# TUMFTM/CamRaDepth

Measured on AMD Instinct MI355X. Metric: training images/sec at 256x416 bf16, higher is better.
Workload: dtype bf16; 1 GPU; CamRaDepth base (image+radar) train step, 8x7x256x416 per GPU, bf16 MFMA / fp32 accumulate, diffGradNorm + OneCycleLR, Dropout2d/DropPath on; global_batch=8, parallelism=dp1, hip_graph=True

## Files before the change

camradepth_amd/csrc/encoder_ops.hip:

```cpp
#include <stdlib.h>
#include "common.h"

namespace {

constexpr int TPB = 256;

constexpr int DTH = 8;
constexpr int DCW = 64;

struct InNorm {
  const crd_sum_t* stats;
  const float* gamma; const float* beta; int gmul;
};
__device__ __forceinline__ void innorm_coeffs(const InNorm& n, int b, int C, long long P, int c0, bool ok, float (&a)[8], float (&s)[8]) {
#pragma unroll
  for (int j = 0; j < 8; ++j) { a[j] = 1.f; s[j] = 0.f; }
  if (n.stats == nullptr || !ok) return;
  float mean, rstd;
  const int grp = (c0 >> 4) / n.gmul;
  gn_mean_rstd(n.stats + (long long)b * (C >> 4) * 2, grp * n.gmul, n.gmul, (float)P * 16.f * n.gmul, mean, rstd);
#pragma unroll
  for (int j = 0; j < 8; ++j) {
    a[j] = n.gamma[c0 + j] * rstd;
    s[j] = n.beta[c0 + j] - mean * a[j];
// ... 32 lines not shown
  bf16_t* yb = y + (long long)b * H * W * C;
  const int t = threadIdx.x;
  const int nG = (C - c_win) >= DCW ? 8 : (C - c_win) >> 3;
  const int g = t & 7, xc = (t >> 3) % TW, rg = (t >> 3) / TW;
  const int c0 = c_win + g * 8;
  const bool gok = g < nG;
  typedef __attribute__((ext_vector_type(2))) float f32x2;
  f32x2 wv[9][4], bv[4];
  {
    uint4 r[(HPX * 8 + TPB - 1) / TPB];
    bool inimg[(HPX * 8 + TPB - 1) / TPB];
#pragma unroll
    for (int k = 0; k < (HPX * 8 + TPB - 1) / TPB; ++k) {
      const int i = t + k * TPB;
      const int hp = i >> 3, g = i & 7;
      const int hy = hp / HWD, hx = hp - hy * HWD;
      const int iy = ty0 - 1 + hy, ix = tx0 - 1 + hx;
      inimg[k] = i < HPX * 8 && g < nG && (unsigned)iy < (unsigned)H && (unsigned)ix < (unsigned)W;
      const int cy = iy < 0 ? 0 : (iy < H ? iy : H - 1), cx = ix < 0 ? 0 : (ix < W ? ix : W - 1), cgr = g < nG ? g : 0;
      const uint4 u = *reinterpret_cast<const uint4*>(xb + ((long long)cy * W + cx) * C + c_win + cgr * 8);
      r[k] = inimg[k] ? u : make_uint4(0, 0, 0, 0);
    }
#pragma unroll
    for (int tp = 0; tp < 9; ++tp) {
      float w8[8];
      if (gok) load8t<1>(w9, (long long)(FLIP ? 8 - tp : tp) * C + c0, w8);
      else {
#pragma unroll
        for (int j = 0; j < 8; ++j) w8[j] = 0.f;
      }
#pragma unroll
      for (int q = 0; q < 4; ++q) wv[tp][q] = f32x2{w8[2 * q], w8[2 * q + 1]};
    }
#pragma unroll
    for (int q = 0; q < 4; ++q) bv[q] = f32x2{(bias && gok) ? bias[c0 + 2 * q] : 0.f, (bias && gok) ? bias[c0 + 2 * q + 1] : 0.f};
    float na[8], ns[8];
    innorm_coeffs(inn, b, C, (long long)H * W, c_win + (t & 7) * 8, (t & 7) < nG, na, ns);
#pragma unroll
    for (int k = 0; k < (HPX * 8 + TPB - 1) / TPB; ++k) {
      const int i = t + k * TPB;
      if (i < HPX * 8) sh[i] = (inn.stats && inimg[k]) ? innorm_apply(r[k], na, ns) : r[k];
    }
  }
  uint4 xrv[ROWS];
  if (red.xr) {
    const int cgr = gok ? c0 : c_win;
#pragma unroll
    for (int i = 0; i < ROWS; ++i) {
      const int oy = ty0 + rg * ROWS + i, ox = tx0 + xc;
      const int cy = oy < H ? oy : H - 1, cx = ox < W ? ox : W - 1;
      xrv[i] = *reinterpret_cast<const uint4*>(red.xr + (((long long)b * H + cy) * W + cx) * C + cgr);
    }
  }
  __syncthreads();
  auto lds8 = [&](int hy, int hx, f32x2 (&v)[4]) {
    const uint4 u = sh[(hy * HWD + hx) * 8 + g];
    v[0] = f32x2{bf_lo(u.x), bf_hi(u.x)}; v[1] = f32x2{bf_lo(u.y), bf_hi(u.y)};
    v[2] = f32x2{bf_lo(u.z), bf_hi(u.z)}; v[3] = f32x2{bf_lo(u.w), bf_hi(u.w)};
  };
  f32x2 win[3][3][4];
  const int r0 = rg * ROWS;
#pragma unroll
  for (int ky = 0; ky < 2; ++ky)
#pragma unroll
    for (int kx = 0; kx < 3; ++kx) lds8(r0 + ky, xc + kx, win[ky][kx]);
  float s = 0.f, ss = 0.f;
  float rs0[8], rs1[8], rmean = 0.f, rrstd = 0.f;
#pragma unroll
  for (int j = 0; j < 8; ++j) rs0[j] = rs1[j] = 0.f;
  if (red.xr && gok) gn_mean_rstd(red.stats + (long long)b * (C >> 4) * 2, c0 >> 4, 1, (float)H * W * 16.f, rmean, rrstd);
#pragma unroll
  for (int i = 0; i < ROWS; ++i) {
#pragma unroll
    for (int kx = 0; kx < 3; ++kx) lds8(r0 + i + 2, xc + kx, win[(i + 2) % 3][kx]);
    const int oy = ty0 + r0 + i, ox = tx0 + xc;
    f32x2 acc[4];
#pragma unroll
    for (int q = 0; q < 4; ++q) acc[q] = bv[q];
#pragma unroll
    for (int ky = 0; ky < 3; ++ky)
#pragma unroll
      for (int kx = 0; kx < 3; ++kx) {
#pragma unroll
        for (int q = 0; q < 4; ++q) acc[q] = __builtin_elementwise_fma(win[(i + ky) % 3][kx][q], wv[ky * 3 + kx][q], acc[q]);
      }
    if (gok && oy < H && ox < W) {
      uint4 u;
      u.x = pack_bf2(acc[0][0], acc[0][1]); u.y = pack_bf2(acc[1][0], acc[1][1]); u.z = pack_bf2(acc[2][0], acc[2][1]); u.w = pack_bf2(acc[3][0], acc[3][1]);
      *reinterpret_cast<uint4*>(yb + ((long long)oy * W + ox) * C + c0) = u;
      if (red.xr) {
        const uint4 xv = xrv[i];
        const float gq[8] = {bf_lo(u.x), bf_hi(u.x), bf_lo(u.y), bf_hi(u.y), bf_lo(u.z), bf_hi(u.z), bf_lo(u.w), bf_hi(u.w)};
        const float xq[8] = {bf_lo(xv.x), bf_hi(xv.x), bf_lo(xv.y), bf_hi(xv.y), bf_lo(xv.z), bf_hi(xv.z), bf_lo(xv.w), bf_hi(xv.w)};
#pragma unroll
        for (int j = 0; j < 8; ++j) { rs0[j] += gq[j]; rs1[j] += gq[j] * ((xq[j] - rmean) * rrstd); }
      }
      if (STATS) {
        s += bf_lo(u.x) + bf_hi(u.x) + bf_lo(u.y) + bf_hi(u.y) + bf_lo(u.z) + bf_hi(u.z) + bf_lo(u.w) + bf_hi(u.w);
        ss += bf_lo(u.x) * bf_lo(u.x) + bf_hi(u.x) * bf_hi(u.x) + bf_lo(u.y) * bf_lo(u.y) + bf_hi(u.y) * bf_hi(u.y) +
              bf_lo(u.z) * bf_lo(u.z) + bf_hi(u.z) * bf_hi(u.z) + bf_lo(u.w) * bf_lo(u.w) + bf_hi(u.w) * bf_hi(u.w);
      }
    }
  }
  if (STATS) {
    s += __shfl_xor(s, 1); ss += __shfl_xor(ss, 1);
#pragma unroll
    for (int o = 8; o < 64; o <<= 1) { s += __shfl_xor(s, o); ss += __shfl_xor(ss, o); }
    const int wave = t >> 6, l = t & 63;
    if (l < 8 && (l & 1) == 0) { sred[wave][(l >> 1) * 2] = s; sred[wave][(l >> 1) * 2 + 1] = ss; }
    __syncthreads();
    if (t < 8) {
      const float v = sred[0][t] + sred[1][t] + sred[2][t] + sred[3][t];
      const int slab = (c_win >> 4) + (t >> 1);
      if (slab < (C >> 4)) stat_add(&stats[((long long)b * (C >> 4) + slab) * 2 + (t & 1)], v);
    }
  }
  if (red.xr) {
#pragma unroll
    for (int o = 8; o < 64; o <<= 1) {
#pragma unroll
      for (int j = 0; j < 8; ++j) { rs0[j] += __shfl_xor(rs0[j], o); rs1[j] += __shfl_xor(rs1[j], o); }
    }
    __syncthreads();
    float* fr = reinterpret_cast<float*>(sh);
    const int wave = t >> 6, l = t & 63;
    if (l < 8) {
#pragma unroll
      for (int j = 0; j < 8; ++j) { fr[wave * 128 + (l * 8 + j) * 2] = rs0[j]; fr[wave * 128 + (l * 8 + j) * 2 + 1] = rs1[j]; }
    }
    __syncthreads();
    const int nch = nG * 8;
    if (t < 2 * nch) {
      const float v = fr[t] + fr[128 + t] + fr[256 + t] + fr[384 + t];
      const int c = c_win + (t >> 1);
      grad_add(&red.r[((long long)b * C + c) * 2 + (t & 1)], v);
      fr[512 + t] = v * red.gamma[c];
    }
    __syncthreads();
    if (t < 2 * (nch >> 4)) {
      const int grp = t >> 1, which = t & 1;
      float a = 0.f;
#pragma unroll
      for (int j = 0; j < 16; ++j) a += fr[512 + (grp * 16 + j) * 2 + which];
      grad_add(&red.r[(long long)gridDim.z * C * 2 + ((long long)b * (C >> 4) + (c_win >> 4) + grp) * 2 + which], a);
    }
  }
}

#ifndef CRD_DWW_WGS
#define CRD_DWW_WGS 2
#endif
template <int TW>
__global__ __launch_bounds__(TPB, CRD_DWW_WGS) void k_dwconv_wgrad(const bf16_t* x, const bf16_t* dy, int H, int W, int C, crd_sum_t* dw10,
                                                      int replicas, int tiles_x, int tiles_y, int tiles_per_wg, InNorm inn) {
  constexpr int HWD = TW + 2;
  constexpr int HPX = (DTH + 2) * HWD;
  constexpr int RSPLIT = 32 / TW;
  constexpr int ROWS = DTH / RSPLIT;
  extern __shared__ __attribute__((aligned(16))) uint4 dsm[];
  uint4* sx = dsm;
  uint4* sdy = dsm + HPX * 8;
  const int b = blockIdx.z;
  const int c_win = blockIdx.y * DCW;
  const int txi = blockIdx.x % tiles_x, ygrp = blockIdx.x / tiles_x;
  const int tx0 = txi * TW;
  const bf16_t* xb = x + (long long)b * H * W * C;
  const bf16_t* db = dy + (long long)b * H * W * C;
  const int t = threadIdx.x;
  const int nG = (C - c_win) >= DCW ? 8 : (C - c_win) >> 3;
  const int g = t & 7, xc = (t >> 3) % TW, rg = (t >> 3) / TW;
  float acc[10][8];
#pragma unroll
  for (int tp = 0; tp < 10; ++tp)
#pragma unroll
    for (int j = 0; j < 8; ++j) acc[tp][j] = 0.f;
  auto unpack8 = [&](const uint4& u, float (&v)[8]) {
    v[0] = bf_lo(u.x); v[1] = bf_hi(u.x); v[2] = bf_lo(u.y); v[3] = bf_hi(u.y);
    v[4] = bf_lo(u.z); v[5] = bf_hi(u.z); v[6] = bf_lo(u.w); v[7] = bf_hi(u.w);
  };
  float na[8], ns[8];
  for (int it = 0; it < tiles_per_wg; ++it) {
    const int tyi = ygrp * tiles_per_wg + it;
    if (tyi >= tiles_y) break;
    const int ty0 = tyi * DTH;
    {
      constexpr int NX = (HPX * 8 + TPB - 1) / TPB, ND = (DTH * TW * 8) / TPB;
      uint4 rx[NX], rd[ND];
      bool inimg[NX];
#pragma unroll
      for (int k = 0; k < NX; ++k) {
        const int i = t + k * TPB;
        const int hp = i >> 3, gg = i & 7;
        const int hy = hp / HWD, hx = hp - hy * HWD;
        const int iy = ty0 - 1 + hy, ix = tx0 - 1 + hx;
        inimg[k] = i < HPX * 8 && gg < nG && (unsigned)iy < (unsigned)H && (unsigned)ix < (unsigned)W;
        const int cy = iy < 0 ? 0 : (iy < H ? iy : H - 1), cx = ix < 0 ? 0 : (ix < W ? ix : W - 1), cgr = gg < nG ? gg : 0;
        const uint4 u = *reinterpret_cast<const uint4*>(xb + ((long long)cy * W + cx) * C + c_win + cgr * 8);
        rx[k] = inimg[k] ? u : make_uint4(0, 0, 0, 0);
      }
#pragma unroll
      for (int k = 0; k < ND; ++k) {
        const int i = t + k * TPB;
        const int pp = i >> 3, gg = i & 7;
        const int py = pp / TW, px = pp - py * TW;
        const int iy = ty0 + py, ix = tx0 + px;
        const int cy = iy < H ? iy : H - 1, cx = ix < W ? ix : W - 1, cgr = gg < nG ? gg : 0;
        const uint4 u = *reinterpret_cast<const uint4*>(db + ((long long)cy * W + cx) * C + c_win + cgr * 8);
        rd[k] = (gg < nG && iy < H && ix < W) ? u : make_uint4(0, 0, 0, 0);
      }
      if (it == 0) innorm_coeffs(inn, b, C, (long long)H * W, c_win + (t & 7) * 8, (t & 7) < nG, na, ns);
      if (it > 0) __syncthreads();
#pragma unroll
      for (int k = 0; k < NX; ++k) {
        const int i = t + k * TPB;
        if (i < HPX * 8) sx[i] = (inn.stats && inimg[k]) ? innorm_apply(rx[k], na, ns) : rx[k];
      }
#pragma unroll
      for (int k = 0; k < ND; ++k) sdy[t + k * TPB] = rd[k];
    }
    __syncthreads();
    float win[3][3][8];
    const int r0 = rg * ROWS;
#pragma unroll
    for (int ky = 0; ky < 2; ++ky)
#pragma unroll
      for (int kx = 0; kx < 3; ++kx) unpack8(sx[((r0 + ky) * HWD + xc + kx) * 8 + g], win[ky][kx]);
#pragma unroll
    for (int i = 0; i < ROWS; ++i) {
#pragma unroll
      for (int kx = 0; kx < 3; ++kx) unpack8(sx[((r0 + i + 2) * HWD + xc + kx) * 8 + g], win[(i + 2) % 3][kx]);
      float d[8];
      unpack8(sdy[((r0 + i) * TW + xc) * 8 + g], d);
#pragma unroll
      for (int j = 0; j < 8; ++j) acc[9][j] += d[j];
#pragma unroll
      for (int ky = 0; ky < 3; ++ky)
#pragma unroll
        for (int kx = 0; kx < 3; ++kx) {
#pragma unroll
          for (int j = 0; j < 8; ++j) acc[ky * 3 + kx][j] += d[j] * win[(i + ky) % 3][kx][j];
        }
    }
  }
#pragma unroll
  for (int o = 8; o < 64; o <<= 1) {
#pragma unroll
    for (int tp = 0; tp < 10; ++tp)
#pragma unroll
      for (int j = 0; j < 8; ++j) acc[tp][j] += __shfl_xor(acc[tp][j], o);
  }
  __syncthreads();
  float* sm = reinterpret_cast<float*>(dsm);
  const int wave = t >> 6, l = t & 63;
  for (int w = 0; w < 4; ++w) {
    if (wave == w && l < 8) {
#pragma unroll
      for (int tp = 0; tp < 10; ++tp)
#pragma unroll
        for (int j = 0; j < 8; ++j) {
          float* p = &sm[tp * 64 + l * 8 + j];
          *p = w == 0 ? acc[tp][j] : *p + acc[tp][j];
        }
    }
    __syncthreads();
  }
  crd_sum_t* dst = dw10 + (long long)((blockIdx.z * gridDim.x + blockIdx.x) % replicas) * 10 * C;
  const int nch = nG * 8;
  for (int i = t; i < 10 * nch; i += TPB) {
    const int tp = i / nch, cl = i - tp * nch;
    const float v = sm[tp * 64 + cl];
    if (v != 0.f) grad_add(&dst[(long long)tp * C + c_win + cl], v);
  }
}

template <class PRE, class F>
__device__ __forceinline__ void matvec_rows(const bf16_t* w, int ld, int r_lo, int r_hi, int ncols, const float* sx, PRE&& pre, F&& out) {
  const int l = threadIdx.x & 63, wave = threadIdx.x >> 6, nw = blockDim.x >> 6;
  auto load_rows = [&](int r0, int c0, float (&wv)[4][8]) {
#pragma unroll
    for (int k = 0; k < 4; ++k) {
      const int r = r0 + k < r_hi ? r0 + k : r_hi - 1;
      load8(w + (long long)r * ld, c0 < ncols ? c0 : 0, 0, wv[k]);
    }
  };
  float w0[4][8];
  const int r_first = r_lo + wave * 4;
  load_rows(r_first < r_hi ? r_first : r_lo, l * 8, w0);
  pre();
  for (int r0 = r_first; r0 < r_hi; r0 += nw * 4) {
    double acc[4] = {0.0, 0.0, 0.0, 0.0};
    for (int c0 = l * 8; c0 < ncols; c0 += 512) {
      float wv[4][8];
      if (r0 == r_first && c0 == l * 8) {
#pragma unroll
        for (int k = 0; k < 4; ++k)
#pragma unroll
          for (int j = 0; j < 8; ++j) wv[k][j] = w0[k][j];
      } else {
        load_rows(r0, c0, wv);
      }
#pragma unroll
      for (int k = 0; k < 4; ++k)
#pragma unroll
        for (int j = 0; j < 8; ++j) acc[k] += (double)wv[k][j] * (double)sx[c0 + j];
    }
#pragma unroll
    for (int k = 0; k < 4; ++k)
#pragma unroll
      for (int o = 32; o > 0; o >>= 1) acc[k] += __shfl_xor(acc[k], o);
    if (l == 0) {
#pragma unroll
      for (int k = 0; k < 4; ++k)
        if (r0 + k < r_hi) out(r0 + k, (float)acc[k]);
    }
  }
}
constexpr int VEC_ROWS = 64;

struct XbarProj { const crd_sum_t* chan; const crd_sum_t* stats; const float* gamma; const float* beta; const bf16_t* w; int N, C; bf16_t* xbar; float* u; };
__device__ __forceinline__ void attn_xbar_proj_body(const XbarProj& x, int b, int e) {
  __shared__ float sx[1024];
  const int C = x.C, N = x.N, nt = blockDim.x;
  const int r_lo = e * VEC_ROWS, r_hi = r_lo + VEC_ROWS < C ? r_lo + VEC_ROWS : C;
  float* ub = x.u + (long long)b * C;
  matvec_rows(x.w, C, r_lo, r_hi, C, sx,
              [&]() {
                for (int c = threadIdx.x; c < C; c += nt) {
                  float mean, rstd;
                  gn_mean_rstd(x.stats + (long long)b * (C >> 4) * 2, c >> 4, 1, (float)N * 16.f, mean, rstd);
                  const float mc = stat_get(&x.chan[((long long)b * C + c) * 2]) / (float)N;
                  const bf16_t q = f2bf(x.gamma[c] * (mc - mean) * rstd + x.beta[c]);
                  if (e == 0) x.xbar[(long long)b * C + c] = q;
                  sx[c] = bf2f(q);
                }
                __syncthreads();
              },
              [&](int r, float v) { ub[r] = v; });
}

__global__ __launch_bounds__(1024) void k_attn_scores(const bf16_t* q, const bf16_t* k, int N, int M, int heads, int d,
                                                      float scale, float* S, short* idx, int qg, XbarProj xp) {
  __shared__ float smax[16][32];
  const int b = blockIdx.y;
  const int nvec = xp.chan ? (xp.C + VEC_ROWS - 1) / VEC_ROWS : 0;
  if ((int)blockIdx.x < nvec) { attn_xbar_proj_body(xp, b, blockIdx.x); return; }
  const int tile_x = blockIdx.x - nvec;
  const int l = threadIdx.x & 63, wave = threadIdx.x >> 6;
  const int h = wave % heads, g = wave / heads;
  const int n0 = (tile_x * qg + g) * 32;
  const int C = heads * d;
  const int n = n0 + (l & 31);
  const bool nok = n < N;
  const bf16_t* qb = q + ((long long)b * N + (nok ? n : 0)) * C;
  const bf16_t* kb = k + (long long)b * M * C;
  const int half = l >> 5;
  bf16x8 qf[4];
#pragma unroll
  for (int ks = 0; ks < 4; ++ks) {
    const int kk = ks * 16 + half * 8;
    uint4 u = *reinterpret_cast<const uint4*>(qb + h * d + (kk < d ? kk : 0));
    if (kk >= d) u = make_uint4(0, 0, 0, 0);
    qf[ks] = *reinterpret_cast<bf16x8*>(&u);
  }
  float best = -INFINITY;
  int besti = 0;
  const bool kcol_ok[4] = {half * 8 < d, 16 + half * 8 < d, 32 + half * 8 < d, 48 + half * 8 < d};
  auto load_keys = [&](int m0, uint4 (&dst)[4]) {
    int mrow = m0 + (l & 31);
    mrow = mrow < M ? mrow : M - 1;
    const bf16_t* rowp = kb + (long long)mrow * C + h * d;
#pragma unroll
    for (int ks = 0; ks < 4; ++ks) dst[ks] = *reinterpret_cast<const uint4*>(rowp + (kcol_ok[ks] ? ks * 16 + half * 8 : 0));
  };
  auto score_tile = [&](int m0, const uint4 (&kt)[4]) {
    f32x16 acc;
#pragma unroll
    for (int r = 0; r < 16; ++r) acc[r] = 0.f;
#pragma unroll
    for (int ks = 0; ks < 4; ++ks) {
      uint4 kf = kt[ks];
      if (!kcol_ok[ks]) kf = make_uint4(0, 0, 0, 0);
      acc = __builtin_amdgcn_mfma_f32_32x32x16_bf16(*reinterpret_cast<const bf16x8*>(&kf), qf[ks], acc, 0, 0, 0);
    }
    const bool edge = m0 + 32 > M;
#pragma unroll
    for (int r = 0; r < 16; r += 2) {
      const int ma = m0 + (r & 3) + 8 * (r >> 2) + 4 * half;
      const uint32_t p1 = pack_bf2(acc[r], acc[r + 1]);
      const uint32_t p2 = pack_bf2(bf_lo(p1) * scale, bf_hi(p1) * scale);
      float va = bf_lo(p2), vb = bf_hi(p2);
      if (edge) { va = ma < M ? va : -INFINITY; vb = ma + 1 < M ? vb : -INFINITY; }
      const bool ta = va > best;
      best = ta ? va : best;
      besti = ta ? ma : besti;
      const bool tb = vb > best;
      best = tb ? vb : best;
      besti = tb ? ma + 1 : besti;
    }
  };
  uint4 ring[4][4];
#pragma unroll
  for (int j = 0; j < 4; ++j) load_keys(j * 32, ring[j]);
  for (int m0 = 0; m0 < M; m0 += 128) {
#pragma unroll
    for (int j = 0; j < 4; ++j) {
      score_tile(m0 + j * 32, ring[j]);
      __builtin_amdgcn_sched_barrier(0);
      load_keys(m0 + j * 32 + 128, ring[j]);
      __builtin_amdgcn_sched_barrier(0);
    }
  }
  float ob = __shfl_xor(best, 32);
  int oi = __shfl_xor(besti, 32);
  if (ob > best || (ob == best && oi < besti)) { best = ob; besti = oi; }
  if (nok && half == 0) idx[((long long)b * N + n) * heads + h] = (short)besti;
  if (half == 0) smax[wave][l] = best;
  __syncthreads();
  if (h == 0 && half == 0 && nok) {
    float Ssum = 0.f;
    for (int hh = 0; hh < heads; ++hh) Ssum += smax[g * heads + hh][l];
    S[(long long)b * N + n] = Ssum;
  }
}

// ... 251 lines not shown
  for (long long i0 = threadIdx.x; i0 < total; i0 += (long long)UB * TPB) {
    int cgv[UB], mv[UB];
    long long nv[UB];
    float gv[UB];
#pragma unroll
    for (int u = 0; u < UB; ++u) {
      const long long i = i0 + (long long)u * TPB;
      const bool ok = i < total;
      cgv[u] = ok ? (int)(i % CG) : 0;
      nv[u] = ok ? p0 + i / CG : p0;
      const int h = (cgv[u] * 8) / d;
      mv[u] = idx[((long long)b * N + nv[u]) * heads + h];
      gv[u] = ok ? scale * dS[(long long)b * N + nv[u]] : 0.f;
    }
    uint4 kraw[UB], qraw[UB];
#pragma unroll
    for (int u = 0; u < UB; ++u) {
      kraw[u] = *reinterpret_cast<const uint4*>(k + ((long long)b * M + mv[u]) * C + cgv[u] * 8);
      qraw[u] = *reinterpret_cast<const uint4*>(q + ((long long)b * N + nv[u]) * C + cgv[u] * 8);
    }
#pragma unroll
    for (int u = 0; u < UB; ++u) {
      if (i0 + (long long)u * TPB >= total) continue;
      float kv[8];
      kv[0] = bf_lo(kraw[u].x); kv[1] = bf_hi(kraw[u].x); kv[2] = bf_lo(kraw[u].y); kv[3] = bf_hi(kraw[u].y);
      kv[4] = bf_lo(kraw[u].z); kv[5] = bf_hi(kraw[u].z); kv[6] = bf_lo(kraw[u].w); kv[7] = bf_hi(kraw[u].w);
#pragma unroll
      for (int j = 0; j < 8; ++j) kv[j] *= gv[u];
      store8_bf16(dq, ((long long)b * N + nv[u]) * C + cgv[u] * 8, kv);
      if (use_lds) {
        const int nl = (int)(nv[u] - p0);
        sq[nl * CG + cgv[u]] = qraw[u];
        const int h = (cgv[u] * 8) / d;
        if (cgv[u] * 8 == h * d) atomicOr(&mask[(h * M + mv[u]) * WPC + (nl >> 5)], 1u << (nl & 31));
        if (cgv[u] == 0) sg[nl] = gv[u];
      } else {
        float qv[8];
        qv[0] = bf_lo(qraw[u].x); qv[1] = bf_hi(qraw[u].x); qv[2] = bf_lo(qraw[u].y); qv[3] = bf_hi(qraw[u].y);
        qv[4] = bf_lo(qraw[u].z); qv[5] = bf_hi(qraw[u].z); qv[6] = bf_lo(qraw[u].w); qv[7] = bf_hi(qraw[u].w);
        crd_sum_t* dst = &dk[((long long)b * M + mv[u]) * C + cgv[u] * 8];
#pragma unroll
        for (int j = 0; j < 8; ++j) grad_add(dst + j, gv[u] * qv[j]);
      }
    }
  }
  if (!use_lds) return;
  __syncthreads();
  float* outp = dk_part ? dk_part + ((long long)chunk_x * gridDim.y + b) * M * C : nullptr;
  for (int pr = threadIdx.x; pr < M * CG; pr += TPB) {
    const int m = pr / CG, cg = pr - m * CG;
    const int h = (cg * 8) / d;
    const unsigned* mk = mask + (h * M + m) * WPC;
    float acc[8];
#pragma unroll
    for (int j = 0; j < 8; ++j) acc[j] = 0.f;
    for (int w = 0; w < WPC; ++w) {
      unsigned bits = mk[w];
      while (bits) {
        const int n = (w << 5) + __builtin_ctz(bits);
        bits &= bits - 1;
        const uint4 u = sq[n * CG + cg];
        const float g = sg[n];
        acc[0] += g * bf_lo(u.x); acc[1] += g * bf_hi(u.x); acc[2] += g * bf_lo(u.y); acc[3] += g * bf_hi(u.y);
        acc[4] += g * bf_lo(u.z); acc[5] += g * bf_hi(u.z); acc[6] += g * bf_lo(u.w); acc[7] += g * bf_hi(u.w);
      }
    }
    if (outp) {
      store8_f32(outp, (long long)m * C + cg * 8, acc);
    } else {
      crd_sum_t* dst = &dk[((long long)b * M + m) * C + cg * 8];
#pragma unroll
      for (int j = 0; j < 8; ++j)
        if (acc[j] != 0.f) grad_add(dst + j, acc[j]);
    }
  }
}

__global__ __launch_bounds__(TPB) void k_sum_partials_bf16(const float* part, int replicas, long long stride, bf16_t* dst, long long n8) {
  for (long long i = (long long)blockIdx.x * TPB + threadIdx.x; i < n8; i += (long long)gridDim.x * TPB) {
    float v[8];
#pragma unroll
    for (int j = 0; j < 8; ++j) v[j] = 0.f;
    for (int r0 = 0; r0 < replicas; r0 += 4) {
      float w[4][8];
#pragma unroll
      for (int k = 0; k < 4; ++k) load8(part, (long long)(r0 + k < replicas ? r0 + k : replicas - 1) * stride + i * 8, 1, w[k]);
#pragma unroll
      for (int k = 0; k < 4; ++k) {
        const bool ok = r0 + k < replicas;
#pragma unroll
        for (int j = 0; j < 8; ++j) v[j] += ok ? w[k][j] : 0.f;
      }
    }
    store8_bf16(dst, i * 8, v);
  }
}

__global__ __launch_bounds__(TPB) void k_gsum_to_bf16(const crd_sum_t* src, bf16_t* dst, long long n8) {
  for (long long i = (long long)blockIdx.x * TPB + threadIdx.x; i < n8; i += (long long)gridDim.x * TPB) {
    float v[8];
#pragma unroll
    for (int j = 0; j < 8; ++j) v[j] = grad_get(src + i * 8 + j);
    store8_bf16(dst, i * 8, v);
  }
}

}

static int dw_tile_width(int W) {
  static int forced = -1;
  if (forced < 0) forced = crd_dev_int("CRD_DW_TW", 0);
  if (forced == 16 || forced == 32) return forced;
  return W <= 16 ? 16 : 32;
}

extern "C" int crd_dwconv3x3(const void* x, int32_t B, int32_t H, int32_t W, int32_t C, const float* w9, const float* bias,
                             int32_t flip, void* y, crd_sum_t* stats, const crd_sum_t* in_stats, int32_t in_gmul,
                             const float* in_gamma, const float* in_beta, const void* red_x, const crd_sum_t* red_stats,
                             const float* red_gamma, crd_sum_t* red_r, crd_stream_t stream) {
  CRD_CHECK_ARG(x && w9 && y, "crd_dwconv3x3: null pointer");
  CRD_CHECK_ARG(!red_x || (red_stats && red_gamma && red_r), "crd_dwconv3x3: incomplete fused-reduce arguments");
  const RedOut red{reinterpret_cast<const bf16_t*>(red_x), red_stats, red_gamma, red_r};
  CRD_CHECK_ARG(!in_stats || (in_gamma && in_beta && in_gmul >= 1 && (C / 16) % in_gmul == 0), "crd_dwconv3x3: bad input-norm arguments");
  const InNorm inn{in_stats, in_gamma, in_beta, in_gmul};
  CRD_CHECK_ARG(C % 16 == 0, "crd_dwconv3x3: C must be a multiple of 16");
  const bf16_t* xp = reinterpret_cast<const bf16_t*>(x);
  bf16_t* yp = reinterpret_cast<bf16_t*>(y);
  hipStream_t st = as_stream(stream);
  const int tw = dw_tile_width(W);
  const int tiles_x = cdiv(W, tw), tiles_y = cdiv(H, DTH);
  dim3 grid(tiles_x * tiles_y, cdiv(C, DCW), B);
#define CRD_DW(FL, STT, TWV) hipLaunchKernelGGL((k_dwconv<FL, STT, TWV>), grid, dim3(TPB), 0, st, xp, H, W, C, w9, bias, yp, stats, tiles_x, inn, red)
  if (tw == 32) {
    if (flip) { if (stats) CRD_DW(true, true, 32); else CRD_DW(true, false, 32); }
    else { if (stats) CRD_DW(false, true, 32); else CRD_DW(false, false, 32); }
  } else {
    if (flip) { if (stats) CRD_DW(true, true, 16); else CRD_DW(true, false, 16); }
    else { if (stats) CRD_DW(false, true, 16); else CRD_DW(false, false, 16); }
  }
#undef CRD_DW
  CRD_LAUNCH_CHECK("crd_dwconv3x3");
  return CRD_OK;
}

extern "C" int crd_dwconv3x3_wgrad(const void* x, const void* dy, int32_t B, int32_t H, int32_t W, int32_t C, crd_sum_t* dw10,
                                   int32_t replicas, const crd_sum_t* in_stats, int32_t in_gmul, const float* in_gamma,
                                   const float* in_beta, crd_stream_t stream) {
  CRD_CHECK_ARG(x && dy && dw10 && replicas >= 1, "crd_dwconv3x3_wgrad: null pointer / replicas < 1");
  CRD_CHECK_ARG(!in_stats || (in_gamma && in_beta && in_gmul >= 1 && (C / 16) % in_gmul == 0), "crd_dwconv3x3_wgrad: bad input-norm arguments");
  const InNorm inn{in_stats, in_gamma, in_beta, in_gmul};
  CRD_CHECK_ARG(C % 16 == 0 && C <= 4096, "crd_dwconv3x3_wgrad: C must be a multiple of 16, <= 4096");
  const int tw = dw_tile_width(W);
  const int tiles_x = cdiv(W, tw), tiles_y = cdiv(H, DTH), wins = cdiv(C, DCW);
  int ysplit = cdiv(512, (long long)tiles_x * wins * B);
  if (ysplit > tiles_y) ysplit = tiles_y;
  if (ysplit < 1) ysplit = 1;
  const int per = cdiv(tiles_y, ysplit);
  ysplit = cdiv(tiles_y, per);
  dim3 grid(tiles_x * ysplit, wins, B);
  const bf16_t* xp = reinterpret_cast<const bf16_t*>(x);
  const bf16_t* dp = reinterpret_cast<const bf16_t*>(dy);
  hipStream_t st = as_stream(stream);
  static bool attr_done[2] = {false, false};
  if (tw == 32) {
    const size_t lds = (size_t)((DTH + 2) * 34 * 8 + DTH * 32 * 8) * sizeof(uint4);
    if (!attr_done[0]) { crd_reserve_lds(reinterpret_cast<const void*>(&k_dwconv_wgrad<32>), (int)lds, "k_dwconv_wgrad"); attr_done[0] = true; }
    hipLaunchKernelGGL(k_dwconv_wgrad<32>, grid, dim3(TPB), lds, st, xp, dp, H, W, C, dw10, replicas, tiles_x, tiles_y, per, inn);
  } else {
    const size_t lds = (size_t)((DTH + 2) * 18 * 8 + DTH * 16 * 8) * sizeof(uint4);
    if (!attr_done[1]) { crd_reserve_lds(reinterpret_cast<const void*>(&k_dwconv_wgrad<16>), (int)lds, "k_dwconv_wgrad"); attr_done[1] = true; }
    hipLaunchKernelGGL(k_dwconv_wgrad<16>, grid, dim3(TPB), lds, st, xp, dp, H, W, C, dw10, replicas, tiles_x, tiles_y, per, inn);
  }
  CRD_LAUNCH_CHECK("crd_dwconv3x3_wgrad");
  return CRD_OK;
}

static int attn_scores_launch(const void* q, const void* k, int32_t B, int32_t N, int32_t M, int32_t heads, int32_t d, float scale,
                              float* S, int16_t* idx, const XbarProj& xp, const char* who, crd_stream_t stream) {
  CRD_CHECK_ARG(q && k && S && idx, "%s: null pointer", who);
  CRD_UNSUPPORTED(d % 8 == 0 && d <= 64 && M < 32768, "%s: head dim must be a multiple of 8, <= 64 (got %d)", who, d);
  CRD_UNSUPPORTED(heads >= 1 && heads <= 16, "%s: at most 16 heads (got %d)", who, heads);
  int qg = 8 / heads;
  if (qg < 1) qg = 1;
  if (qg > 4) qg = 4;
  dim3 grid(cdiv(N, 32 * qg) + (xp.chan ? cdiv(xp.C, VEC_ROWS) : 0), B);
  hipLaunchKernelGGL(k_attn_scores, grid, dim3(64 * heads * qg), 0, as_stream(stream), reinterpret_cast<const bf16_t*>(q),
                     reinterpret_cast<const bf16_t*>(k), N, M, heads, d, scale, S, idx, qg, xp);
  CRD_LAUNCH_CHECK(who);
  return CRD_OK;
}

extern "C" int crd_attn_scores(const void* q, const void* k, int32_t B, int32_t N, int32_t M, int32_t heads, int32_t d,
                               float scale, float* S, int16_t* idx, crd_stream_t stream) {
  return attn_scores_launch(q, k, B, N, M, heads, d, scale, S, idx, XbarProj{}, "crd_attn_scores", stream);
}

extern "C" int crd_attn_scores_fp8(const void* q8, const void* k8, int32_t B, int32_t N, int32_t M, int32_t heads, float qk_scale,
                                   float scale, float* ssum, int16_t* idx, crd_stream_t stream) {
  CRD_CHECK_ARG(q8 && k8 && ssum && idx && B > 0 && N > 0 && M > 0 && qk_scale > 0.f, "crd_attn_scores_fp8: bad argument");
  CRD_UNSUPPORTED(heads >= 1 && heads <= 16, "crd_attn_scores_fp8: at most 16 heads");
  CRD_CHECK_ARG((reinterpret_cast<uintptr_t>(q8) & 15) == 0 && (reinterpret_cast<uintptr_t>(k8) & 15) == 0, "crd_attn_scores_fp8: 16-byte aligned operands");
  int qg = 8 / heads;
  if (qg < 1) qg = 1;
  if (qg > 4) qg = 4;
  hipLaunchKernelGGL(k_attn_scores_fp8, dim3(cdiv(N, 32 * qg), B), dim3(64 * heads * qg), 0, as_stream(stream),
                     reinterpret_cast<const unsigned char*>(q8), reinterpret_cast<const unsigned char*>(k8), N, M, heads, qk_scale, scale, ssum,
                     reinterpret_cast<short*>(idx), qg);
  CRD_LAUNCH_CHECK("crd_attn_scores_fp8");
  return CRD_OK;
}

extern "C" int crd_attn_fwd(const void* q, const void* k, int32_t B, int32_t N, int32_t M, int32_t heads, int32_t d, float scale,
                            float* S, int16_t* idx, const crd_sum_t* chan_sums, const crd_sum_t* stats, const float* gamma,
                            const float* beta, const void* w_fwd, void* xbar, float* u, crd_stream_t stream) {
  CRD_CHECK_ARG(chan_sums && stats && gamma && beta && w_fwd && xbar && u, "crd_attn_fwd: null pointer");
  const int C = heads * d;
  CRD_UNSUPPORTED(C % 16 == 0 && C <= 1024, "crd_attn_fwd: C must be a multiple of 16, <= 1024");
  return attn_scores_launch(q, k, B, N, M, heads, d, scale, S, idx,
                            XbarProj{chan_sums, stats, gamma, beta, reinterpret_cast<const bf16_t*>(w_fwd), N, C,
                                     reinterpret_cast<bf16_t*>(xbar), u}, "crd_attn_fwd", stream);
}

extern "C" int crd_attn_xbar(const crd_sum_t* chan_sums, const crd_sum_t* stats, const float* gamma, const float* beta, int32_t B,
                             int32_t N, int32_t C, void* xbar, crd_stream_t stream) {
  CRD_CHECK_ARG(chan_sums && stats && gamma && beta && xbar, "crd_attn_xbar: null pointer");
  hipLaunchKernelGGL(k_attn_xbar, dim3(B), dim3(256), 0, as_stream(stream), chan_sums, stats, gamma, beta, N, C,
                     reinterpret_cast<bf16_t*>(xbar));
  CRD_LAUNCH_CHECK("crd_attn_xbar");
  return CRD_OK;
}

extern "C" int crd_attn_xbar_proj(const crd_sum_t* chan_sums, const crd_sum_t* stats, const float* gamma, const float* beta, const void* w_fwd,
                                  int32_t B, int32_t N, int32_t C, void* xbar, float* u, crd_stream_t stream) {
  CRD_CHECK_ARG(chan_sums && stats && gamma && beta && w_fwd && xbar && u, "crd_attn_xbar_proj: null pointer");
  CRD_UNSUPPORTED(C % 16 == 0 && C <= 1024, "crd_attn_xbar_proj: C must be a multiple of 16, <= 1024");
  hipLaunchKernelGGL(k_attn_xbar_proj, dim3(cdiv(C, VEC_ROWS), B), dim3(TPB), 0, as_stream(stream),
                     XbarProj{chan_sums, stats, gamma, beta, reinterpret_cast<const bf16_t*>(w_fwd), N, C, reinterpret_cast<bf16_t*>(xbar), u});
  CRD_LAUNCH_CHECK("crd_attn_xbar_proj");
  return CRD_OK;
}

extern "C" int crd_attn_vec_bwd(const crd_sum_t* t, const void* w_dgrad, int32_t B, int32_t C, int32_t Cpad, float inv_n, void* tb, float* es,
                                crd_stream_t stream) {
  CRD_CHECK_ARG(t && w_dgrad && tb && es, "crd_attn_vec_bwd: null pointer");
  CRD_UNSUPPORTED(C % 8 == 0 && C <= 1024 && Cpad >= C && Cpad % 8 == 0, "crd_attn_vec_bwd: C must be a multiple of 8, <= 1024");
  hipLaunchKernelGGL(k_attn_vec_bwd, dim3(cdiv(C, VEC_ROWS), B), dim3(TPB), 0, as_stream(stream),
                     VecBwd{t, reinterpret_cast<const bf16_t*>(w_dgrad), C, Cpad, inv_n, reinterpret_cast<bf16_t*>(tb), es});
  CRD_LAUNCH_CHECK("crd_attn_vec_bwd");
  return CRD_OK;
}

extern "C" int crd_attn_out_residual(const float* x, const float* u, const float* S, const float* bp, const float* dp,
                                     int32_t B, int32_t N, int32_t C, float* x1, crd_stream_t stream) {
  CRD_CHECK_ARG(x && u && S && bp && x1, "crd_attn_out_residual: null pointer");
  CRD_CHECK_ARG(C % 8 == 0, "crd_attn_out_residual: C %% 8");
  const long long total = (long long)N * (C / 8);
  int nblk = cdiv(total, TPB);
  if (nblk > 2048) nblk = 2048;
  hipLaunchKernelGGL(k_attn_out_residual, dim3(nblk, B), dim3(TPB), 0, as_stream(stream), x, u, S, bp, dp, (long long)N, C, x1);
  CRD_LAUNCH_CHECK("crd_attn_out_residual");
  return CRD_OK;
}

static int attn_out_bwd_launch(float* dx1, const float* u, const float* S, const float* dp, int32_t B, int32_t N, int32_t C, crd_sum_t* t,
                               crd_sum_t* dbp_rows, float* dS, const GnPre* pre, const char* who, crd_stream_t stream) {
  CRD_CHECK_ARG(dx1 && u && S && t && dbp_rows && dS, "%s: null pointer", who);
  CRD_UNSUPPORTED(C % 8 == 0 && C <= 512, "%s: C must be a multiple of 8 and <= 512", who);
  static int small = -1;
  if (small < 0) small = crd_dev_int("CRD_ATTN_OUT_BWD_CHUNK", 32);
  int nblk = cdiv(N, (long long)B * cdiv(N, 256) < 128 ? small : 256);
  int cap = 1024 / (B > 0 ? B : 1); if (cap < 1) cap = 1;
  if (nblk > cap) nblk = cap;
  int chunk = cdiv(N, nblk);
  nblk = cdiv(N, chunk);
  if (pre) hipLaunchKernelGGL(k_attn_out_bwd<true>, dim3(nblk, B), dim3(TPB), 2 * C * sizeof(float), as_stream(stream), dx1, u, S, dp,
                              (long long)N, C, chunk, t, dbp_rows, dS, *pre);
  else hipLaunchKernelGGL(k_attn_out_bwd<false>, dim3(nblk, B), dim3(TPB), 2 * C * sizeof(float), as_stream(stream), dx1, u, S, dp,
                          (long long)N, C, chunk, t, dbp_rows, dS, GnPre{});
  CRD_LAUNCH_CHECK(who);
  return CRD_OK;
}

extern "C" int crd_attn_out_bwd(const float* dx1, const float* u, const float* S, const float* dp, int32_t B, int32_t N,
                                int32_t C, crd_sum_t* t, crd_sum_t* dbp_rows, float* dS, crd_stream_t stream) {
  return attn_out_bwd_launch(const_cast<float*>(dx1), u, S, dp, B, N, C, t, dbp_rows, dS, nullptr, "crd_attn_out_bwd", stream);
}

extern "C" int crd_attn_out_bwd_gn(float* dx1, const float* u, const float* S, const float* dp, int32_t B, int32_t N, int32_t C,
                                   crd_sum_t* t, crd_sum_t* dbp_rows, float* dS, const float* x, const void* dxn, const crd_sum_t* stats,
                                   const float* gamma, const crd_sum_t* r, float* dgamma, float* dbeta, crd_stream_t stream) {
  CRD_CHECK_ARG(x && dxn && stats && gamma && r, "crd_attn_out_bwd_gn: null pointer");
  CRD_CHECK_ARG(C % 16 == 0 && (dgamma == nullptr) == (dbeta == nullptr), "crd_attn_out_bwd_gn: C %% 16, dgamma / dbeta both or neither");
  const GnPre pre{x, reinterpret_cast<const bf16_t*>(dxn), stats, gamma, r, dgamma, dbeta, B};
  return attn_out_bwd_launch(dx1, u, S, dp, B, N, C, t, dbp_rows, dS, &pre, "crd_attn_out_bwd_gn", stream);
}

static size_t attn_bwd_lds(int chunk, int M, int heads, int C) {
  return (size_t)chunk * C * 2 + (size_t)chunk * 4 + (size_t)heads * M * ((chunk + 31) / 32) * 4 + 16;
}
static int attn_bwd_blocks(int B, int N, int M, int heads, int C) {
  static int small = -1, mid = -1;
  if (small < 0) {
    small = crd_dev_int("CRD_ATTN_BWD_CHUNK", 32);
    mid = crd_dev_int("CRD_ATTN_BWD_CHUNK2", 64);
  }
  int target = 128;
  if ((long long)B * cdiv(N, 128) < 128) target = N <= 512 ? small : mid;
  int nblk = cdiv(N, target);
  int cap = 2048 / (B > 0 ? B : 1); if (cap < 1) cap = 1;
  if (nblk > cap) nblk = cap;
  const int chunk = cdiv(N, nblk);
  if (attn_bwd_lds(chunk, M, heads, C) > 128 * 1024 || chunk > 32767) return 0;
  return cdiv(N, chunk);
}

extern "C" int crd_attn_scores_bwd_partials(int32_t B, int32_t N, int32_t M, int32_t heads, int32_t d) {
  return attn_bwd_blocks(B, N, M, heads, heads * d);
}

static int attn_scores_bwd_launch(const void* q, const void* k, const float* dS, const int16_t* idx, int32_t B, int32_t N,
                                  int32_t M, int32_t heads, int32_t d, float scale, void* dq, crd_sum_t* dk, float* dk_partials,
                                  const VecBwd& vec, const char* who, crd_stream_t stream) {
  CRD_CHECK_ARG(q && k && dS && idx && dq && (dk || dk_partials), "%s: null pointer", who);
  CRD_CHECK_ARG(d % 8 == 0, "%s: head dim must be a multiple of 8", who);
// ... 63 lines not shown
```

Baseline: 458.8 images/s.

## Restructure depthwise conv weight-grad kernel with prefetch pipelining and flattened batch tiling

Rewrites the depthwise 3x3 weight-gradient kernel so each workgroup walks a flattened list of (batch, x-tile, y-tile) items. It prefetches the next tile's input and dy into registers while computing the current one, and per-batch norm coefficients are staged in LDS. The accumulation uses packed float2 FMAs, and the cross-wave reduction writes per-wave partials once instead of looping four serialized barrier rounds. Batch is folded into grid.x so fewer workgroups emit atomics, at the cost of more register pressure and more complex index math.

Result: no change. 460.9 images/s (median of 4 runs) (+0.5%).

```diff
diff --git a/camradepth_amd/csrc/encoder_ops.hip b/camradepth_amd/csrc/encoder_ops.hip
--- a/camradepth_amd/csrc/encoder_ops.hip
+++ b/camradepth_amd/csrc/encoder_ops.hip
@@ -208,124 +208,171 @@
 #endif
 template <int TW>
 __global__ __launch_bounds__(TPB, CRD_DWW_WGS) void k_dwconv_wgrad(const bf16_t* x, const bf16_t* dy, int H, int W, int C, crd_sum_t* dw10,
-                                                      int replicas, int tiles_x, int tiles_y, int tiles_per_wg, InNorm inn) {
+                                                      int replicas, int tiles_x, int tiles_y, int n_items, int tiles_per_wg, InNorm inn) {
   constexpr int HWD = TW + 2;
   constexpr int HPX = (DTH + 2) * HWD;
   constexpr int RSPLIT = 32 / TW;
   constexpr int ROWS = DTH / RSPLIT;
+  constexpr int NXB = (DTH + 2) / RSPLIT, NX = NXB + 1, ND = DTH / RSPLIT;
+  constexpr bool DY_EARLY = TW == 16;
+  typedef __attribute__((ext_vector_type(2))) float f32x2;
   extern __shared__ __attribute__((aligned(16))) uint4 dsm[];
   uint4* sx = dsm;
   uint4* sdy = dsm + HPX * 8;
-  const int b = blockIdx.z;
   const int c_win = blockIdx.y * DCW;
-  const int txi = blockIdx.x % tiles_x, ygrp = blockIdx.x / tiles_x;
-  const int tx0 = txi * TW;
-  const bf16_t* xb = x + (long long)b * H * W * C;
-  const bf16_t* db = dy + (long long)b * H * W * C;
   const int t = threadIdx.x;
   const int nG = (C - c_win) >= DCW ? 8 : (C - c_win) >> 3;
   const int g = t & 7, xc = (t >> 3) % TW, rg = (t >> 3) / TW;
-  float acc[10][8];
+  const bool gok = g < nG;
+  const int tiles = tiles_x * tiles_y;
+  const int q0 = blockIdx.x * tiles_per_wg;
+  const int q1 = q0 + tiles_per_wg < n_items ? q0 + tiles_per_wg : n_items;
+  f32x2 acc[10][4];
 #pragma unroll
   for (int tp = 0; tp < 10; ++tp)
 #pragma unroll
-    for (int j = 0; j < 8; ++j) acc[tp][j] = 0.f;
-  auto unpack8 = [&](const uint4& u, float (&v)[8]) {
-    v[0] = bf_lo(u.x); v[1] = bf_hi(u.x); v[2] = bf_lo(u.y); v[3] = bf_hi(u.y);
-    v[4] = bf_lo(u.z); v[5] = bf_hi(u.z); v[6] = bf_lo(u.w); v[7] = bf_hi(u.w);
+    for (int j = 0; j < 4; ++j) acc[tp][j] = f32x2{0.f, 0.f};
+  auto unpack8 = [&](const uint4& u, f32x2 (&v)[4]) {
+    v[0] = f32x2{bf_lo(u.x), bf_hi(u.x)}; v[1] = f32x2{bf_lo(u.y), bf_hi(u.y)};
+    v[2] = f32x2{bf_lo(u.z), bf_hi(u.z)}; v[3] = f32x2{bf_lo(u.w), bf_hi(u.w)};
   };
-  float na[8], ns[8];
-  for (int it = 0; it < tiles_per_wg; ++it) {
-    const int tyi = ygrp * tiles_per_wg + it;
-    if (tyi >= tiles_y) break;
-    const int ty0 = tyi * DTH;
-    {
-      constexpr int NX = (HPX * 8 + TPB - 1) / TPB, ND = (DTH * TW * 8) / TPB;
-      uint4 rx[NX], rd[ND];
-      bool inimg[NX];
-#pragma unroll
-      for (int k = 0; k < NX; ++k) {
-        const int i = t + k * TPB;
-        const int hp = i >> 3, gg = i & 7;
-        const int hy = hp / HWD, hx = hp - hy * HWD;
-        const int iy = ty0 - 1 + hy, ix = tx0 - 1 + hx;
-        inimg[k] = i < HPX * 8 && gg < nG && (unsigned)iy < (unsigned)H && (unsigned)ix < (unsigned)W;
-        const int cy = iy < 0 ? 0 : (iy < H ? iy : H - 1), cx = ix < 0 ? 0 : (ix < W ? ix : W - 1), cgr = gg < nG ? gg : 0;
-        const uint4 u = *reinterpret_cast<const uint4*>(xb + ((long long)cy * W + cx) * C + c_win + cgr * 8);
-        rx[k] = inimg[k] ? u : make_uint4(0, 0, 0, 0);
-      }
-#pragma unroll
-      for (int k = 0; k < ND; ++k) {
-        const int i = t + k * TPB;
-        const int pp = i >> 3, gg = i & 7;
-        const int py = pp / TW, px = pp - py * TW;
-        const int iy = ty0 + py, ix = tx0 + px;
-        const int cy = iy < H ? iy : H - 1, cx = ix < W ? ix : W - 1, cgr = gg < nG ? gg : 0;
-        const uint4 u = *reinterpret_cast<const uint4*>(db + ((long long)cy * W + cx) * C + c_win + cgr * 8);
-        rd[k] = (gg < nG && iy < H && ix < W) ? u : make_uint4(0, 0, 0, 0);
-      }
-      if (it == 0) innorm_coeffs(inn, b, C, (long long)H * W, c_win + (t & 7) * 8, (t & 7) < nG, na, ns);
-      if (it > 0) __syncthreads();
-#pragma unroll
-      for (int k = 0; k < NX; ++k) {
-        const int i = t + k * TPB;
-        if (i < HPX * 8) sx[i] = (inn.stats && inimg[k]) ? innorm_apply(rx[k], na, ns) : rx[k];
-      }
-#pragma unroll
-      for (int k = 0; k < ND; ++k) sdy[t + k * TPB] = rd[k];
-    }
+  const int lane_c = c_win + (gok ? g : 0) * 8;
+  const int eh = t >> 4, ew = TW + ((t >> 3) & 1);
+  uint4 rx[NX], rd[ND];
+  bool mxc, mec, mdc;
+  int ty0 = 0;
+  auto request = [&](int q, bool live, bool want_x, bool want_dy) {
+    const int b = q / tiles, rem = q - b * tiles;
+    const int txi = rem / tiles_y, tyi = rem - txi * tiles_y;
+    const int tx0 = txi * TW;
+    ty0 = tyi * DTH;
+    const long long img = live ? (long long)b * H * W : 0ll;
+    auto col = [&](int ix, bool& ok) {
+      ok = gok && (unsigned)ix < (unsigned)W;
+      const int cx = ix < 0 ? 0 : (ix < W ? ix : W - 1);
+      return (live ? cx * C : 0) + lane_c;
+    };
+    auto row = [&](const bf16_t* p, int iy) {
+      const int cy = iy < 0 ? 0 : (iy < H ? iy : H - 1);
+      return p + (img + (live ? (long long)cy * W : 0ll)) * C;
+    };
+    if (want_x) {
+      const int ox = col(tx0 - 1 + xc, mxc), oe = col(tx0 - 1 + ew, mec);
+#pragma unroll
+      for (int k = 0; k < NXB; ++k) rx[k] = *reinterpret_cast<const uint4*>(row(x, ty0 - 1 + RSPLIT * k + rg) + ox);
+      rx[NXB] = *reinterpret_cast<const uint4*>(row(x, ty0 - 1 + (eh < DTH + 2 ? eh : 0)) + oe);
+    }
+    if (want_dy) {
+      const int od = col(tx0 + xc, mdc);
+#pragma unroll
+      for (int k = 0; k < ND; ++k) rd[k] = *reinterpret_cast<const uint4*>(row(dy, ty0 + RSPLIT * k + rg) + od);
+    }
+  };
+  float* scoef = reinterpret_cast<float*>(sdy + DTH * TW * 8);
+  auto coeffs = [&](int b) {
+    float a8[8], s8[8];
+    innorm_coeffs(inn, b, C, (long long)H * W, c_win + g * 8, gok, a8, s8);
+    if (t < 8) {
+#pragma unroll
+      for (int j = 0; j < 8; ++j) { scoef[t * 16 + j] = a8[j]; scoef[t * 16 + 8 + j] = s8[j]; }
+    }
+  };
+  auto to_lds = [&]() {
+    auto keep = [](bool c, const uint4& v) { return make_uint4(c ? v.x : 0u, c ? v.y : 0u, c ? v.z : 0u, c ? v.w : 0u); };
+    float na[8], ns[8];
+    if (inn.stats) {
+#pragma unroll
+      for (int j = 0; j < 8; ++j) { na[j] = scoef[g * 16 + j]; ns[j] = scoef[g * 16 + 8 + j]; }
+    }
+    auto put = [&](int hy, int hx, bool cok, uint4 v) {
+      if (inn.stats) v = innorm_apply(v, na, ns);
+      sx[(hy * HWD + hx) * 8 + g] = keep(cok && (unsigned)(ty0 - 1 + hy) < (unsigned)H, v);
+    };
+#pragma unroll
+    for (int k = 0; k < NXB; ++k) put(RSPLIT * k + rg, xc, mxc, rx[k]);
+    if (eh < DTH + 2) put(eh, ew, mec, rx[NXB]);
+#pragma unroll
+    for (int k = 0; k < ND; ++k) {
+      const int py = RSPLIT * k + rg;
+      sdy[(py * TW + xc) * 8 + g] = keep(mdc && ty0 + py < H, rd[k]);
+    }
+  };
+  request(q0, true, true, true);
+  int b_cur = q0 / tiles;
+  if (inn.stats) { coeffs(b_cur); __syncthreads(); }
+  to_lds();
+  __syncthreads();
+  const int r0 = rg * ROWS;
+  for (int q = q0;; ++q) {
+    const bool more = q + 1 < q1;
+    request(more ? q + 1 : q, more, true, DY_EARLY);
+    __builtin_amdgcn_sched_barrier(0);
+#ifndef CRD_DWW_NO_COMPUTE
+    f32x2 d[3][4];
+#pragma unroll
+    for (int hy = 0; hy < ROWS + 2; ++hy) {
+      f32x2 xr[3][4];
+#pragma unroll
+      for (int kx = 0; kx < 3; ++kx) unpack8(sx[((r0 + hy) * HWD + xc + kx) * 8 + g], xr[kx]);
+      if (hy < ROWS) {
+        unpack8(sdy[((r0 + hy) * TW + xc) * 8 + g], d[hy % 3]);
+#pragma unroll
+        for (int j = 0; j < 4; ++j) acc[9][j] += d[hy % 3][j];
+      }
+#pragma unroll
+      for (int ky = 2; ky >= 0; --ky) {
+        const int o = hy - ky;
+        if (o < 0 || o >= ROWS) continue;
+#pragma unroll
+        for (int kx = 0; kx < 3; ++kx)
+#pragma unroll
+          for (int j = 0; j < 4; ++j) acc[ky * 3 + kx][j] = __builtin_elementwise_fma(d[o % 3][j], xr[kx][j], acc[ky * 3 + kx][j]);
+      }
+    }
+#endif
+    __builtin_amdgcn_sched_barrier(0);
+    if (!more) break;
+    const int bn = (q + 1) / tiles;
+    if (inn.stats && bn != b_cur) {
+      b_cur = bn;
+      coeffs(b_cur);
+    }
+    if (!DY_EARLY) request(q + 1, true, false, true);
     __syncthreads();
-    float win[3][3][8];
-    const int r0 = rg * ROWS;
-#pragma unroll
-    for (int ky = 0; ky < 2; ++ky)
-#pragma unroll
-      for (int kx = 0; kx < 3; ++kx) unpack8(sx[((r0 + ky) * HWD + xc + kx) * 8 + g], win[ky][kx]);
-#pragma unroll
-    for (int i = 0; i < ROWS; ++i) {
-#pragma unroll
-      for (int kx = 0; kx < 3; ++kx) unpack8(sx[((r0 + i + 2) * HWD + xc + kx) * 8 + g], win[(i + 2) % 3][kx]);
-      float d[8];
-      unpack8(sdy[((r0 + i) * TW + xc) * 8 + g], d);
-#pragma unroll
-      for (int j = 0; j < 8; ++j) acc[9][j] += d[j];
-#pragma unroll
-      for (int ky = 0; ky < 3; ++ky)
-#pragma unroll
-        for (int kx = 0; kx < 3; ++kx) {
-#pragma unroll
-          for (int j = 0; j < 8; ++j) acc[ky * 3 + kx][j] += d[j] * win[(i + ky) % 3][kx][j];
-        }
-    }
+    to_lds();
+    __syncthreads();
   }
 #pragma unroll
   for (int o = 8; o < 64; o <<= 1) {
 #pragma unroll
     for (int tp = 0; tp < 10; ++tp)
 #pragma unroll
-      for (int j = 0; j < 8; ++j) acc[tp][j] += __shfl_xor(acc[tp][j], o);
+      for (int j = 0; j < 4; ++j) {
+        acc[tp][j][0] += __shfl_xor(acc[tp][j][0], o);
+        acc[tp][j][1] += __shfl_xor(acc[tp][j][1], o);
+      }
   }
   __syncthreads();
   float* sm = reinterpret_cast<float*>(dsm);
   const int wave = t >> 6, l = t & 63;
-  for (int w = 0; w < 4; ++w) {
-    if (wave == w && l < 8) {
-#pragma unroll
-      for (int tp = 0; tp < 10; ++tp)
-#pragma unroll
-        for (int j = 0; j < 8; ++j) {
-          float* p = &sm[tp * 64 + l * 8 + j];
-          *p = w == 0 ? acc[tp][j] : *p + acc[tp][j];
-        }
-    }
-    __syncthreads();
-  }
-  crd_sum_t* dst = dw10 + (long long)((blockIdx.z * gridDim.x + blockIdx.x) % replicas) * 10 * C;
+  if (l < 8) {
+#pragma unroll
+    for (int tp = 0; tp < 10; ++tp)
+#pragma unroll
+      for (int j = 0; j < 4; ++j) *reinterpret_cast<f32x2*>(&sm[wave * 640 + tp * 64 + l * 8 + 2 * j]) = acc[tp][j];
+  }
+  __syncthreads();
+  crd_sum_t* dst = dw10 + (long long)((blockIdx.y * gridDim.x + blockIdx.x) % replicas) * 10 * C;
   const int nch = nG * 8;
   for (int i = t; i < 10 * nch; i += TPB) {
     const int tp = i / nch, cl = i - tp * nch;
-    const float v = sm[tp * 64 + cl];
+    const int k = tp * 64 + cl;
+    const float v = (sm[k] + sm[640 + k]) + (sm[1280 + k] + sm[1920 + k]);
+#ifdef CRD_DWW_NO_ATOMICS
+    if (v == 12345.678f) grad_add(&dst[(long long)tp * C + c_win + cl], v);
+#else
     if (v != 0.f) grad_add(&dst[(long long)tp * C + c_win + cl], v);
+#endif
   }
 }
 
@@ -883,24 +930,26 @@
   CRD_CHECK_ARG(C % 16 == 0 && C <= 4096, "crd_dwconv3x3_wgrad: C must be a multiple of 16, <= 4096");
   const int tw = dw_tile_width(W);
   const int tiles_x = cdiv(W, tw), tiles_y = cdiv(H, DTH), wins = cdiv(C, DCW);
-  int ysplit = cdiv(512, (long long)tiles_x * wins * B);
-  if (ysplit > tiles_y) ysplit = tiles_y;
-  if (ysplit < 1) ysplit = 1;
-  const int per = cdiv(tiles_y, ysplit);
-  ysplit = cdiv(tiles_y, per);
-  dim3 grid(tiles_x * ysplit, wins, B);
+  CRD_UNSUPPORTED((long long)B * tiles_x * tiles_y < (1ll << 30), "crd_dwconv3x3_wgrad: %lld tiles", (long long)B * tiles_x * tiles_y);
+  const int n_items = B * tiles_x * tiles_y;
+  int slots = 512 / wins;
+  if (slots > n_items) slots = n_items;
+  if (slots < 1) slots = 1;
+  const int per = cdiv(n_items, slots);
+  slots = cdiv(n_items, per);
+  dim3 grid(slots, wins);
   const bf16_t* xp = reinterpret_cast<const bf16_t*>(x);
   const bf16_t* dp = reinterpret_cast<const bf16_t*>(dy);
   hipStream_t st = as_stream(stream);
   static bool attr_done[2] = {false, false};
   if (tw == 32) {
-    const size_t lds = (size_t)((DTH + 2) * 34 * 8 + DTH * 32 * 8) * sizeof(uint4);
+    const size_t lds = (size_t)((DTH + 2) * 34 * 8 + DTH * 32 * 8) * sizeof(uint4) + 512;
     if (!attr_done[0]) { crd_reserve_lds(reinterpret_cast<const void*>(&k_dwconv_wgrad<32>), (int)lds, "k_dwconv_wgrad"); attr_done[0] = true; }
-    hipLaunchKernelGGL(k_dwconv_wgrad<32>, grid, dim3(TPB), lds, st, xp, dp, H, W, C, dw10, replicas, tiles_x, tiles_y, per, inn);
+    hipLaunchKernelGGL(k_dwconv_wgrad<32>, grid, dim3(TPB), lds, st, xp, dp, H, W, C, dw10, replicas, tiles_x, tiles_y, n_items, per, inn);
   } else {
-    const size_t lds = (size_t)((DTH + 2) * 18 * 8 + DTH * 16 * 8) * sizeof(uint4);
+    const size_t lds = (size_t)((DTH + 2) * 18 * 8 + DTH * 16 * 8) * sizeof(uint4) + 512;
     if (!attr_done[1]) { crd_reserve_lds(reinterpret_cast<const void*>(&k_dwconv_wgrad<16>), (int)lds, "k_dwconv_wgrad"); attr_done[1] = true; }
-    hipLaunchKernelGGL(k_dwconv_wgrad<16>, grid, dim3(TPB), lds, st, xp, dp, H, W, C, dw10, replicas, tiles_x, tiles_y, per, inn);
+    hipLaunchKernelGGL(k_dwconv_wgrad<16>, grid, dim3(TPB), lds, st, xp, dp, H, W, C, dw10, replicas, tiles_x, tiles_y, n_items, per, inn);
   }
   CRD_LAUNCH_CHECK("crd_dwconv3x3_wgrad");
   return CRD_OK;
```
